# jimmyshe/liorf

Measured on AMD Instinct MI355X. Metric: LM iterations/sec (64-line scan vs 200k-pt map), higher is better.
Workload: dtype f32; 1 GPU; kitti64: 120000-pt scan vs 200000-pt local surf map, 30 LM iterations per scan (early exit off), one scan per GPU at a time, 8 distinct seeded scans in rotation, map replicated; n_q=120000, n_m=200000, distinct_scans=8, parallelism=scan-per-gpu x1

## Files before the change

include/liorf_s2m_debug.h:

```cpp
#ifndef LIORF_S2M_DEBUG_H
#define LIORF_S2M_DEBUG_H

#include "liorf_s2m.h"

#ifdef __cplusplus
extern "C" {
#endif

int  s2m_debug_device_trig(s2m_handle h, const float* x, size_t n, float* s, float* c, float* a);
int  s2m_debug_deferred(s2m_handle h, int slot);
int  s2m_time_iteration_kernel(s2m_handle h, const float pose[6], int reps, float* ms_per_launch);
int  s2m_time_iterations(s2m_handle h, const float pose[6], int reps, float* ms_per_iter, int cap);

int  s2m_time_loop_launches(s2m_handle h, const float pose[6], int reps, float* us_per_launch);

int  s2m_debug_time_steady(s2m_handle h, const float pose[6], int reps, int solve_prev, float* us_per_launch);

#define S2M_PROF_WORDS 32
int  s2m_debug_wave_profile(s2m_handle h, const float pose[6], int launches, uint64_t* out, size_t cap_waves);

int  s2m_debug_device_hypot(s2m_handle h, const float* x, const float* y, size_t n, float* r);

typedef struct s2m_debug_lm_close_out {
    float   AtA[36], AtB[6];
    int32_t n_sel_last;
    s2m_iter_trace trace;
    float   pose[6];
    float   pose_next[6];
    int32_t iters_run, converged, done, stalled, is_degenerate;
    int32_t n_rows_active;
    float   matP[36];
} s2m_debug_lm_close_out;
int  s2m_debug_lm_close(s2m_handle h, int form, int iter, const double* rows, int n_rows, const float pose0[6],
                        int degen_in, const float matP_in[36], s2m_debug_lm_close_out* out);
int  s2m_debug_lm_close_check_args(int form, int iter, int max_iter, const double* rows, int n_rows, const float pose0[6],
                                   const float matP_in[36], const s2m_debug_lm_close_out* out);

#define S2M_DEBUG_PREP_READ   (-1)
#define S2M_DEBUG_PREP_NEW    0
#define S2M_DEBUG_PREP_LEGACY 1
int  s2m_debug_scan_prep(s2m_handle h, int32_t chain, const float pose[6], int32_t* qperm, float* qxyz, int32_t* chunk_parts,
                         int32_t* chunk_factor, int32_t* wave_table, int32_t* n_waves);

#define S2M_ICP_RANGE 8
int  s2m_debug_icp_nearest(s2m_handle h, const void* src, size_t n_src, const void* tgt, size_t n_tgt, size_t stride_bytes, int32_t mode,
                           uint64_t* keys, int32_t* n_fallback);
int  s2m_debug_icp_time_nearest(s2m_handle h, const void* src, size_t n_src, const void* tgt, size_t n_tgt, size_t stride_bytes, int32_t mode,
                                int32_t reps, uint64_t* keys, int32_t* n_fallback, float* us_build, float* us_search);
int  s2m_debug_icp_align_device(s2m_handle h, const void* src, size_t n_src, const void* tgt, size_t n_tgt, size_t stride_bytes,
                                const s2m_icp_params* p , s2m_icp_result* out);
int  s2m_debug_icp_tuning(s2m_handle h, float cell_in_leaves, int32_t shell_cap, int32_t use_grid);

int  s2m_debug_pg_rebase(const double a_launch[12], const double a_now[12], double X[12]);

int  s2m_debug_pg_set_estimate(s2m_handle h, int32_t key, const double X[12]);
int  s2m_debug_pg_linearize(s2m_handle h, int32_t n_variables, int32_t n_extra, double* rc, double* Binv, double* Aof, double* Ji, double* Jj,
                            double* rx, double* ferr, double* fw, double* err, double* wmin);
#define S2M_DEBUG_PG_FWD 0
#define S2M_DEBUG_PG_BWD 1
#define S2M_DEBUG_PG_K   2
#define S2M_DEBUG_PG_KT  3
int  s2m_debug_pg_apply(s2m_handle h, int32_t op, int32_t cols, const double* in, double* out);
int  s2m_debug_pg_apply_check_args(int32_t n_variables, int32_t n_extra, int32_t op, int32_t cols, const double* in, const double* out);
typedef struct s2m_debug_pg_cg_out {
    double  rr, bb;
    int32_t iters, stop;
// ... 9 lines not shown
```

liorf_amd/csrc/s2m_abi_debug.hip:

```cpp
#include <hip/hip_runtime.h>

#include <cmath>
#include <cstring>
#include <algorithm>
#include <limits>
#include <vector>

#include "s2m_context.hpp"
#include "s2m_device.hpp"

using namespace s2m;
using namespace s2m::host;

namespace s2m {

__global__ __launch_bounds__(256) void k_debug_sincos(const float* __restrict__ x, int n, float* __restrict__ s, float* __restrict__ c,
                                                      float* __restrict__ a)
{
    const int i = blockIdx.x * blockDim.x + threadIdx.x;
    if (i < n) { s[i] = glibc_sincosf(x[i], 0); c[i] = glibc_sincosf(x[i], 1); if (a) a[i] = glibc_atanf(x[i]); }
}

__global__ __launch_bounds__(256) void k_debug_hypot(const float* __restrict__ x, const float* __restrict__ y, int n, float* __restrict__ r)
{
// ... 246 lines not shown
    }
    if ((!pose || chain == S2M_DEBUG_PREP_READ) && chunk_factor)
        S2M_HIP(h, hipMemcpyAsync(chunk_factor, h->reg.chunk_factor.p, sizeof(int32_t) * (size_t)n_chunks, hipMemcpyDeviceToHost, h->stream));
    if (qperm) S2M_HIP(h, hipMemcpyAsync(qperm, h->reg.qperm.p, sizeof(int32_t) * n, hipMemcpyDeviceToHost, h->stream));
    if (qxyz) {
        S2M_HIP(h, hipMemcpyAsync(qxyz, h->reg.qx.p, sizeof(float) * n, hipMemcpyDeviceToHost, h->stream));
        S2M_HIP(h, hipMemcpyAsync(qxyz + n, h->reg.qy.p, sizeof(float) * n, hipMemcpyDeviceToHost, h->stream));
        S2M_HIP(h, hipMemcpyAsync(qxyz + 2 * n, h->reg.qz.p, sizeof(float) * n, hipMemcpyDeviceToHost, h->stream));
    }
    if (chunk_parts) S2M_HIP(h, hipMemcpyAsync(chunk_parts, h->reg.chunk_parts.p, sizeof(int32_t) * (size_t)n_chunks, hipMemcpyDeviceToHost, h->stream));
    int32_t nw = 0;
    const bool have_table = !h->reg.table_stale;
    if (have_table) S2M_HIP(h, hipMemcpyAsync(&nw, h->reg.n_waves.p, sizeof(nw), hipMemcpyDeviceToHost, h->stream));
    S2M_HIP(h, hipStreamSynchronize(h->stream));
    if (nw < 0 || nw > h->hctx.table_cap) return fail(h, S2M_ERR_HIP, "wave count outside the table");
    if (wave_table && nw > 0) {
        S2M_HIP(h, hipMemcpyAsync(wave_table, h->reg.wave_table.p, sizeof(int2) * (size_t)nw, hipMemcpyDeviceToHost, h->stream));
        S2M_HIP(h, hipStreamSynchronize(h->stream));
    }
    if (n_waves) *n_waves = have_table ? nw : -1;
    return S2M_OK;
}

int s2m_debug_deferred(s2m_handle h, int slot)
{
    if (!h) return S2M_ERR_INVALID_ARG;
    if (slot >= 0) { if (slot >= (int)h->batch.kids.size()) return S2M_ERR_INVALID_ARG; h = h->batch.kids[(size_t)slot]; }
    return h->reg.h_state ? h->reg.h_state[1].deferred_total : 0;
}

static int time_iterations_impl(s2m_handle h, const float pose[6], int reps, float* ms_mean, float* ms_per_iter)
{
    if (!h || !pose || reps < 1) return S2M_ERR_INVALID_ARG;
    if (!h->reg.have_scan || h->reg.n_m == 0 || h->reg.n_q == 0) return fail(h, S2M_ERR_NO_SCAN, "needs a resident scan and map");
    S2M_HIP(h, hipSetDevice(h->device));
    int rc;
    if ((rc = upload_ctx(h))) return rc;
    const int nit = h->prm.max_iter;
    if (h->reg.iter_events.size() < (size_t)(2 * nit)) {
        const size_t old = h->reg.iter_events.size();
        h->reg.iter_events.resize(2 * nit);
        for (size_t k = old; k < h->reg.iter_events.size(); k++) S2M_HIP(h, hipEventCreate(&h->reg.iter_events[k]));
    }
    std::vector<double> per_iter((size_t)nit, 0.0);
    for (int rep = 0; rep < reps; rep++) {
        S2M_HIP(h, hipMemsetAsync(h->reg.cert.p, 0, sizeof(float4) * h->reg.n_q, h->stream));
// ... 88 lines not shown
```

liorf_amd/csrc/s2m_kernels.hpp:

```cpp
#pragma once
#include "s2m_device.hpp"

namespace s2m {

struct CtxHead { int32_t nblocks, n_q; const int2* wave_table; double* partials; const float *qx, *qy, *qz; float4 *cert, *plane_cache; };
struct StateHead { int32_t done, n_waves, isDegenerate, T_valid; float pose[6]; };
struct LmParams { int32_t min_corr, early_exit; double conv_deg, conv_cm; };
template <bool kPin = true>
__device__ __forceinline__ void load_heads(CtxP cp, gptr<DevState> st, int slot, CtxHead& c, StateHead& s, int& a0, int& a1)
{
    c.nblocks = cp->nblocks; c.n_q = cp->n_q; c.wave_table = cp->wave_table; c.partials = cp->partials;
    c.qx = cp->qx; c.qy = cp->qy; c.qz = cp->qz; c.cert = cp->cert; c.plane_cache = cp->plane_cache;
    s.done = st->done; s.n_waves = st->n_waves; s.isDegenerate = st->isDegenerate; s.T_valid = st->T_valid;
#pragma unroll
    for (int k = 0; k < 6; k++) s.pose[k] = st->pose2[slot][k];
    if (kPin)
    asm volatile("" : "+s"(c.nblocks), "+s"(c.n_q), "+s"(c.wave_table), "+s"(c.partials), "+s"(c.qx), "+s"(c.qy), "+s"(c.qz),
                      "+s"(c.cert), "+s"(c.plane_cache), "+s"(s.done), "+s"(s.n_waves), "+s"(s.isDegenerate), "+s"(s.T_valid),
                      "+s"(s.pose[0]), "+s"(s.pose[1]), "+s"(s.pose[2]), "+s"(s.pose[3]), "+s"(s.pose[4]), "+s"(s.pose[5]), "+s"(a0), "+s"(a1));
}
__device__ __forceinline__ LmParams lm_params(CtxP cp)
{
    LmParams p;
    p.min_corr = cp->min_corr; p.early_exit = cp->early_exit; p.conv_deg = cp->conv_deg; p.conv_cm = cp->conv_cm;
    return p;
}
__device__ __forceinline__ void swap_if(bool c, float& a, float& b)
{
    float t = a; a = c ? b : a; b = c ? t : b;
}
__device__ __forceinline__ void swap_if(bool c, int& a, int& b)
{
    int t = a; a = c ? b : a; b = c ? t : b;
}

__device__ __forceinline__ void chunk_table_body(const int32_t* __restrict__ parts, int n, int n_chunks, int capacity,
                                                 int2* __restrict__ table, int32_t* __restrict__ n_waves_out,
                                                 int32_t* __restrict__ factor, DevState* __restrict__ st)
{
    __shared__ int32_t wsum[16];
    __shared__ int32_t carry_s, tot_s[3], base_s, pol_s[9];
    const int lane = threadIdx.x & 63, wave = threadIdx.x >> 6;
    constexpr int kOnePerCu = 256 * (kBlock / 64);
    bool use_factor = factor != nullptr;
    if (use_factor) {
        int tb = 0, tf = 0;
        for (int c = threadIdx.x; c < n_chunks; c += 1024) { tb += min(8, parts[c]); tf += min(8, parts[c] * max(factor[c], 1)); }
#pragma unroll
        for (int off = 32; off > 0; off >>= 1) { tb += __shfl_xor(tb, off, 64); tf += __shfl_xor(tf, off, 64); }
        if (threadIdx.x == 0) { tot_s[0] = 0; base_s = 0; }
        __syncthreads();
        if (lane == 0) { atomicAdd(&base_s, tb); atomicAdd(&tot_s[0], tf); }
        __syncthreads();
        use_factor = !(base_s <= kOnePerCu && tot_s[0] > kOnePerCu);
        __syncthreads();
    }
    constexpr int kPolicies = 9;
    auto wish_under = [&](int c, int pol) {
        const int f = use_factor ? max(factor[c], 1) : 1;
        const bool heavy = f >= 8;
        const int fe = (pol == 0) ? f : ((pol == 1) ? (f >= 4 ? f : 1) : (heavy ? f : 1));
        const int w = min(8, parts[c] * fe);
        const int cap = (pol <= 2) ? 8 : ((pol <= 5) ? (heavy ? 8 : (32 >> pol)) : (256 >> pol));
        return min(w, cap);
    };
    int tp[kPolicies];
#pragma unroll
    for (int k = 0; k < kPolicies; k++) tp[k] = 0;
    for (int c = threadIdx.x; c < n_chunks; c += 1024) {
#pragma unroll
        for (int k = 0; k < kPolicies; k++) tp[k] += wish_under(c, k);
    }
#pragma unroll
    for (int k = 0; k < kPolicies; k++) {
#pragma unroll
        for (int off = 32; off > 0; off >>= 1) tp[k] += __shfl_xor(tp[k], off, 64);
    }
    if (threadIdx.x == 0) carry_s = 0;
    if (threadIdx.x < kPolicies) pol_s[threadIdx.x] = 0;
    __syncthreads();
    if (lane == 0) {
#pragma unroll
        for (int k = 0; k < kPolicies; k++) atomicAdd(&pol_s[k], tp[k]);
    }
    __syncthreads();
    const int cap_eff = capacity;
    int pol = kPolicies - 1;
#pragma unroll
    for (int k = kPolicies - 2; k >= 0; k--) if (pol_s[k] <= cap_eff) pol = k;
    auto wish = [&](int c) { return wish_under(c, pol); };
    constexpr int pcap = 8;
    for (int base = 0; base < n_chunks; base += 1024) {
        const int c = base + threadIdx.x;
        const int p = (c < n_chunks) ? min(wish(c), pcap) : 0;
        int incl = p;
#pragma unroll
        for (int off = 1; off < 64; off <<= 1) {
            const int o = __shfl_up(incl, off, 64);
            if (lane >= off) incl += o;
        }
        if (lane == 63) wsum[wave] = incl;
        __syncthreads();
        int woff = 0;
        for (int w = 0; w < wave; w++) woff += wsum[w];
        const int carry = carry_s;
        const int off0 = carry + woff + incl - p;
        if (c < n_chunks) {
            const int per = 64 / p;
            for (int j = 0; j < p; j++) {
                const int start = c * 64 + j * per;
                if (off0 + j < capacity) table[off0 + j] = make_int2(start, max(0, min(per, n - start)));
            }
        }
        __syncthreads();
        if (threadIdx.x == 1023) carry_s = carry + woff + incl;
        __syncthreads();
    }
    if (threadIdx.x == 0) {
        const int nw = min(carry_s, capacity);
        *n_waves_out = nw;
        if (st) st->n_waves = nw;
    }
    if (factor) for (int c = threadIdx.x; c < n_chunks; c += 1024) factor[c] = 0;
}

__global__ __launch_bounds__(1024) void k_chunk_table(const PrepTable tbl)
{
    const PrepSlot& ps = tbl.s[blockIdx.y];
    if (ps.n <= 0) return;
    chunk_table_body(ps.chunk_parts, ps.n, ps.n_chunks, ps.capacity, ps.wave_table, ps.n_waves, nullptr, nullptr);
    if (ps.stamps) {
        __syncthreads();
        if (threadIdx.x == 0) ps.stamps[1] = wall_clock64();
    }
}

__global__ __launch_bounds__(1024) void k_chunk_table_density(const SlotTable tbl)
{
    DevCtx* __restrict__ cp = const_cast<DevCtx*>(tbl.ctx[blockIdx.y]);
    DevState* __restrict__ st = tbl.st[blockIdx.y];
    if (!cp->density_pending) return;
    __syncthreads();
    if (threadIdx.x == 0) cp->density_pending = 0;
    chunk_table_body(cp->chunk_parts, cp->n_q, cp->n_chunks, cp->table_cap, cp->wave_table_rw, cp->n_waves_rw,
                     cp->chunk_factor, st);
}

__device__ __forceinline__ void plane_fit_5x3(float (&qr)[5][3], float (&x)[3])
{
    float hC[3], nU[3], nD[3];
    int perm[3] = { 0, 1, 2 };
#pragma unroll
    for (int k = 0; k < 3; k++) {
        float s = 0.0f;
#pragma unroll
        for (int i = 0; i < 5; i++) s += qr[i][k] * qr[i][k];
        nD[k] = sqrtf(s); nU[k] = nD[k];
    }
    float maxn = nU[0];
    if (nU[1] > maxn) maxn = nU[1];
    if (nU[2] > maxn) maxn = nU[2];
    const float th = maxn * FLT_EPSILON;
    const float threshold_helper = (th * th) / 5.0f;
    const float norm_downdate_threshold = sqrtf(FLT_EPSILON);
    int np = 3;

#pragma unroll
    for (int k = 0; k < 3; k++) {
// ... 406 lines not shown
    if (kFull && iter == 0) {
        __syncthreads();
        if (wave == 1 && lane == 0 && (int)sh.tot[27] >= lp.min_corr) {
            int degenerate = 0;
            if (!all_eigen_above(sh.AtA, cp->eig_thresh)) {
                for (int i = 0; i < 6; i++) for (int j = 0; j < 6; j++) sh.eA[i][j] = sh.AtA[i * 6 + j];
                eigen6_sym(sh.eA, sh.eV, sh.eW, sh.eR, sh.eC);
                for (int i = 0; i < 6; i++) for (int j = 0; j < 6; j++) sh.eV2[i][j] = sh.eV[i][j];
                for (int i = 5; i >= 0; i--) {
                    if (sh.eW[i] < cp->eig_thresh) { for (int j = 0; j < 6; j++) sh.eV2[i][j] = 0.0f; degenerate = 1; }
                    else break;
                }
                for (int i = 0; i < 6; i++) for (int j = 0; j < 6; j++) sh.eA[i][j] = sh.eV[i][j];
                inv6_lu(sh.eA, sh.eVi);
                for (int i = 0; i < 6; i++) for (int j = 0; j < 6; j++) {
                    double a = 0.0;
                    for (int k = 0; k < 6; k++) a += (double)sh.eVi[i][k] * (double)sh.eV2[k][j];
                    st->matP[i * 6 + j] = (float)a;
                }
            }
            st->isDegenerate = degenerate;
            __threadfence_block();
        }
        __syncthreads();
    }

    if (wave == 0) {
        if (n_sel < lp.min_corr) {
            if (t == 0) {
                if (writer) {
                    s2m_iter_trace tr;
                    tr.n_sel = n_sel; tr.stepped = 0; tr.deltaR = 0.0f; tr.deltaT = 0.0f;
#pragma unroll
                    for (int k = 0; k < 6; k++) { tr.pose[k] = pose0[k]; tr.delta[k] = 0.0f; st->pose[k] = pose0[k]; }
                    st->stalled = 1; st->done = 1;
                    st->iters_run = cp->max_iter;
                    store_trace(trace + iter, tr);
                }
#pragma unroll
                for (int k = 0; k < 6; k++) s_out[k] = pose0[k];
                s_out[6] = 1.0f;
            }
        } else {
            float colv[6], X[6];
#pragma unroll
            for (int i = 0; i < 6; i++) colv[i] = (lane < 6) ? sh.AtA[i * 6 + lane] : ((lane == 6) ? sh.AtB[i] : 0.0f);
            solve6_qr_lanes(lane, colv, X);
            if (stamps) stamps[2] = wall_clock64();
            if (t == 0) {
// ... 13 lines not shown
#pragma unroll
                for (int k = 0; k < 6; k++) { pose[k] += X[k]; s_out[k] = pose[k]; }
                const double r0 = (double)(X[0] * 57.29578f), r1 = (double)(X[1] * 57.29578f), r2 = (double)(X[2] * 57.29578f);
                const float deltaR = (float)sqrt(r0 * r0 + r1 * r1 + r2 * r2);
                const double t0 = (double)(X[3] * 100), t1 = (double)(X[4] * 100), t2 = (double)(X[5] * 100);
                const float deltaT = (float)sqrt(t0 * t0 + t1 * t1 + t2 * t2);
                const bool conv = ((double)deltaR < lp.conv_deg) && ((double)deltaT < lp.conv_cm);
                s_out[6] = (conv && lp.early_exit) ? 1.0f : 0.0f;
                if (writer) {
                    s2m_iter_trace tr;
                    tr.n_sel = n_sel; tr.stepped = 1; tr.deltaR = deltaR; tr.deltaT = deltaT;
#pragma unroll
                    for (int k = 0; k < 6; k++) { tr.delta[k] = X[k]; tr.pose[k] = pose[k]; }
#pragma unroll
                    for (int k = 0; k < 6; k++) { st->pose[k] = pose[k]; st->pose2[(iter + 1) & 1][k] = pose[k]; }
                    st->T_valid = 0;
                    store_trace(trace + iter, tr);
                    st->iters_run = iter + 1;
                    if (conv) st->converged = 1;
                    if (conv && lp.early_exit) st->done = 1;
                }
            }
        }
    }
    if (stamps) stamps[3] = wall_clock64();
    late();
    __syncthreads();
    if (stamps) stamps[4] = wall_clock64();
#pragma unroll
    for (int k = 0; k < 6; k++) pose_out[k] = s_out[k];
    return s_out[6] != 0.0f;
}

__global__ __launch_bounds__(256) void k_wave_density(const SlotTable tbl, int raw_limit)
{
    const CtxP cp = ctx_const(tbl.ctx[blockIdx.y]);
    const auto st = G((const DevState*)tbl.st[blockIdx.y]);
    const int lane = threadIdx.x & 63;
    const int wv = blockIdx.x * 4 + (threadIdx.x >> 6);
    if (!cp->density_pending || wv >= st->n_waves) return;
    const auto tb = G((const int2*)cp->wave_table);
    const int2 e = make_int2(tb[wv].x, tb[wv].y);
    const int i = e.x + lane;
    const bool valid = lane < e.y && i < cp->n_q;
    float sx = 0.0f, sy = 0.0f, sz = 0.0f;
    if (valid) {
// ... 215 lines not shown
```

liorf_amd/csrc/s2m_prep.hpp:

```cpp
#pragma once
#include "s2m_device.hpp"

namespace s2m {

__global__ __launch_bounds__(256) void k_bbox(const unsigned char* __restrict__ pts, size_t stride, int n, uint32_t* __restrict__ part)
{
    __shared__ float smn[4][3], smx[4][3];
    float mn[3] = { INFINITY, INFINITY, INFINITY }, mx[3] = { -INFINITY, -INFINITY, -INFINITY };
    for (int i = blockIdx.x * blockDim.x + threadIdx.x; i < n; i += gridDim.x * blockDim.x) {
        const float* p = reinterpret_cast<const float*>(pts + (size_t)i * stride);
#pragma unroll
        for (int d = 0; d < 3; d++) {
            float v = p[d];
            if (isfinite(v)) { mn[d] = fminf(mn[d], v); mx[d] = fmaxf(mx[d], v); }
        }
    }
#pragma unroll
    for (int d = 0; d < 3; d++) {
#pragma unroll
        for (int off = 32; off > 0; off >>= 1) {
            mn[d] = fminf(mn[d], __shfl_down(mn[d], off, 64));
            mx[d] = fmaxf(mx[d], __shfl_down(mx[d], off, 64));
        }
    }
// ... 108 lines not shown
    for (int k = t; k < kPolarCells; k += kPolarBlock) row[k] = hist[k];
}

__global__ __launch_bounds__(1024) void k_polar_prefix(const PrepTable tbl)
{
    const PrepSlot& ps = tbl.s[blockIdx.y];
    if (ps.n <= 0) return;
    int32_t* __restrict__ H = ps.block_hist; const int nb = ps.npb; int32_t* __restrict__ counts = ps.counts;
    __shared__ int32_t seg[16][64];
    const int lane = threadIdx.x & 63, s = threadIdx.x >> 6;
    const int col = blockIdx.x * 64 + lane;
    const int per = (nb + 15) / 16, b0 = min(s * per, nb), b1 = min(b0 + per, nb);
    int32_t sum = 0;
    for (int b = b0; b < b1; b++) sum += H[(size_t)b * kPolarCells + col];
    seg[s][lane] = sum;
    __syncthreads();
    int32_t run = 0, total = 0;
#pragma unroll
    for (int q = 0; q < 16; q++) { const int32_t v = seg[q][lane]; run += (q < s) ? v : 0; total += v; }
    if (s == 0) counts[col] = total;
    for (int b = b0; b < b1; b++) {
        const size_t at = (size_t)b * kPolarCells + col;
        const int32_t v = H[at];
        H[at] = run;
        run += v;
    }
}

__global__ __launch_bounds__(1024) void k_polar_scan(const PrepTable tbl)
{
    const PrepSlot& ps = tbl.s[blockIdx.y];
    if (ps.n <= 0) return;
    int32_t* __restrict__ counts = ps.counts; int32_t* __restrict__ start = ps.cell_start;
    __shared__ int32_t wsum[16];
    const int t = threadIdx.x, lane = t & 63, wave = t >> 6;
    int32_t v[16];
    int32_t sum = 0;
    int4* c4 = reinterpret_cast<int4*>(counts + t * 16);
#pragma unroll
    for (int k = 0; k < 4; k++) {
        const int4 q = c4[k];
        c4[k] = make_int4(0, 0, 0, 0);
        v[4 * k] = q.x; v[4 * k + 1] = q.y; v[4 * k + 2] = q.z; v[4 * k + 3] = q.w;
        sum += q.x + q.y + q.z + q.w;
    }
    int32_t incl = sum;
#pragma unroll
// ... 269 lines not shown
```

liorf_amd/s2m.py:

```python
from __future__ import annotations

import ctypes as C
import importlib.util
import os
import sys

import numpy as np

_HERE = os.path.dirname(os.path.abspath(__file__))
LIB_PATH = os.environ.get("S2M_LIB") or os.path.join(_HERE, "libliorf_s2m.so")

S2M_OK = 0
S2M_ERR_CAPACITY = -5
S2M_ERR_BUSY = -6
ERRORS = {-1: "S2M_ERR_INVALID_ARG", -2: "S2M_ERR_NO_DEVICE", -3: "S2M_ERR_HIP", -4: "S2M_ERR_NO_SCAN",
          -5: "S2M_ERR_CAPACITY", -6: "S2M_ERR_BUSY"}

ABI_SYMBOLS = [
    "s2m_version", "s2m_default_params", "s2m_create", "s2m_destroy", "s2m_last_error", "s2m_set_params", "s2m_get_params",
    "s2m_set_map", "s2m_set_map_device", "s2m_set_scan", "s2m_set_scan_device",
    "s2m_optimize", "s2m_optimize_resident", "s2m_optimize_launch", "s2m_optimize_collect",
    "s2m_optimize_batch", "s2m_batch_set_scan", "s2m_batch_set_scans", "s2m_slot_set_scan", "s2m_slot_optimize_launch", "s2m_slot_optimize_collect", "s2m_optimize_batch_launch", "s2m_optimize_batch_collect", "s2m_batch_get_trace",
    "s2m_get_trace", "s2m_surf_optimization", "s2m_normal_eq", "s2m_last_timing", "s2m_debug_deferred",
    "s2m_time_iteration_kernel", "s2m_time_iterations", "s2m_make_scancontext", "s2m_debug_wave_profile", "s2m_debug_time_steady", "s2m_time_loop_launches",
    "s2m_debug_scan_prep",
    "s2m_voxel_downsample", "s2m_voxel_downsample_device", "s2m_downsample_scan", "s2m_extract_cloud",
    "s2m_transform_cloud",
    "s2m_icp_default_params", "s2m_icp_align", "s2m_debug_device_trig", "s2m_debug_device_hypot",
    "s2m_debug_lm_close", "s2m_debug_lm_close_check_args",
    "s2m_sc_reset", "s2m_sc_size", "s2m_sc_add_scan", "s2m_sc_add_descriptor", "s2m_sc_detect_loop", "s2m_sc_distance",
    "s2m_sc_query_default_params", "s2m_sc_query_check_args", "s2m_sc_query_key", "s2m_sc_query_descriptor", "s2m_sc_query_scan", "s2m_sc_query_projected",
    "s2m_kf_default_params", "s2m_kf_reset", "s2m_kf_size", "s2m_kf_add", "s2m_kf_set_poses", "s2m_extract_surrounding",
    "s2m_loop_default_params", "s2m_loop_near_keyframes", "s2m_loop_align", "s2m_loop_closure_rs",
    "s2m_loop_align_launch", "s2m_loop_closure_rs_launch", "s2m_loop_poll", "s2m_loop_collect",
    "s2m_debug_icp_nearest", "s2m_debug_icp_time_nearest", "s2m_debug_icp_align_device", "s2m_debug_icp_tuning",
    "s2m_gmap_default_params", "s2m_global_map", "s2m_kf_map_cloud",
    "s2m_scan_layout_preset", "s2m_project_default_params", "s2m_imu_deskew_info", "s2m_project_check_args", "s2m_project_scan",
    "s2m_downsample_projected", "s2m_sc_add_projected",
    "s2m_odom_deskew_info", "s2m_project_check_args_motion", "s2m_project_scan_motion", "s2m_guess_state_init", "s2m_update_initial_guess",
    "s2m_pg_default_params", "s2m_pg_check_args", "s2m_pg_reset", "s2m_pg_size", "s2m_pg_add_prior", "s2m_pg_add_between", "s2m_pg_add_gps",
    "s2m_pg_set_initial", "s2m_pg_add_odometry", "s2m_pg_optimize", "s2m_pg_get_poses", "s2m_pg_marginal", "s2m_pg_apply_to_store",
    "s2m_pg_marginals_check_args", "s2m_pg_marginals", "s2m_pg_joint_marginal",
    "s2m_pg_optimize_launch", "s2m_pg_optimize_poll", "s2m_pg_optimize_collect", "s2m_debug_pg_rebase",
    "s2m_debug_pg_set_estimate", "s2m_debug_pg_linearize", "s2m_debug_pg_apply", "s2m_debug_pg_apply_check_args", "s2m_debug_pg_cg",
    "s2m_debug_pg_retract",
]
S2M_RING_U8, S2M_RING_U16, S2M_RING_I32 = 0, 1, 2
S2M_TIME_F32, S2M_TIME_U32_NS, S2M_TIME_U32, S2M_TIME_F64_REL = 0, 1, 2, 3
# ... 195 lines not shown
    L.s2m_optimize_launch.argtypes = [vp, fp]
    L.s2m_optimize_collect.argtypes = [vp, fp, C.POINTER(ImuInit), C.POINTER(Result)]
    L.s2m_get_trace.argtypes = [vp, C.POINTER(IterTrace), C.c_int]
    L.s2m_optimize_batch.argtypes = [vp, C.c_int, C.POINTER(vp), C.POINTER(C.c_size_t), C.c_size_t, fp, C.POINTER(ImuInit), C.POINTER(Result)]
    L.s2m_batch_set_scan.argtypes = [vp, C.c_int, vp, C.c_size_t, C.c_size_t, C.c_int]
    L.s2m_slot_set_scan.argtypes = [vp, C.c_int, vp, C.c_size_t, C.c_size_t, C.c_int]
    L.s2m_slot_optimize_launch.argtypes = [vp, C.c_int, fp]
    L.s2m_slot_optimize_collect.argtypes = [vp, C.c_int, fp, C.POINTER(ImuInit), C.POINTER(Result)]
    L.s2m_batch_set_scans.argtypes = [vp, C.c_int, C.POINTER(C.c_void_p), C.POINTER(C.c_size_t), C.c_size_t, C.c_int]
    L.s2m_optimize_batch_launch.argtypes = [vp, C.c_int, fp]
    L.s2m_optimize_batch_collect.argtypes = [vp, C.c_int, fp, C.POINTER(ImuInit), C.POINTER(Result)]
    L.s2m_batch_get_trace.argtypes = [vp, C.c_int, C.POINTER(IterTrace), C.c_int]
    L.s2m_surf_optimization.argtypes = [vp, fp, C.POINTER(C.c_int32), fp, C.POINTER(C.c_uint8), fp]
    L.s2m_normal_eq.argtypes = [vp, fp, fp, fp, C.POINTER(C.c_int32)]
    L.s2m_last_timing.argtypes = [vp, fp, fp, fp]
    L.s2m_debug_deferred.argtypes = [vp, C.c_int]
    L.s2m_time_iteration_kernel.argtypes = [vp, fp, C.c_int, fp]
    L.s2m_time_iterations.argtypes = [vp, fp, C.c_int, fp, C.c_int]
    L.s2m_debug_wave_profile.argtypes = [vp, fp, C.c_int, C.POINTER(C.c_uint64), C.c_size_t]
    L.s2m_debug_time_steady.argtypes = [vp, fp, C.c_int, C.c_int, fp]
    L.s2m_time_loop_launches.argtypes = [vp, fp, C.c_int, fp]
    L.s2m_debug_scan_prep.argtypes = [vp, C.c_int32, fp, C.POINTER(C.c_int32), fp, C.POINTER(C.c_int32), C.POINTER(C.c_int32),
                                      C.POINTER(C.c_int32), C.POINTER(C.c_int32)]
    L.s2m_make_scancontext.argtypes = [vp, vp, C.c_size_t, C.c_size_t, C.POINTER(C.c_double), C.POINTER(C.c_double)]
    szp = C.POINTER(C.c_size_t)
    for n in ("s2m_voxel_downsample", "s2m_voxel_downsample_device"):
        getattr(L, n).argtypes = [vp, vp, C.c_size_t, C.c_size_t, C.c_float, vp, C.c_size_t, C.c_size_t, szp]
    L.s2m_downsample_scan.argtypes = [vp, vp, C.c_size_t, C.c_size_t, C.c_int, C.c_float, vp, C.c_size_t, C.c_size_t, szp]
    L.s2m_extract_cloud.argtypes = [vp, C.c_int, C.POINTER(vp), szp, C.c_size_t, C.c_int, fp, C.c_float,
                                    vp, C.c_size_t, C.c_size_t, szp]
    L.s2m_transform_cloud.argtypes = [vp, vp, C.c_size_t, C.c_size_t, fp, vp, C.c_size_t]
    dp, i32p = C.POINTER(C.c_double), C.POINTER(C.c_int32)
    L.s2m_debug_device_trig.argtypes = [vp, fp, C.c_size_t, fp, fp, fp]
    L.s2m_debug_device_hypot.argtypes = [vp, fp, fp, C.c_size_t, fp]
    L.s2m_debug_lm_close.argtypes = [vp, C.c_int, C.c_int, dp, C.c_int, fp, C.c_int, fp, C.POINTER(LmCloseOut)]
    L.s2m_debug_lm_close_check_args.argtypes = [C.c_int, C.c_int, C.c_int, dp, C.c_int, fp, fp, C.POINTER(LmCloseOut)]
    L.s2m_icp_default_params.argtypes = [C.POINTER(IcpParams)]
    L.s2m_icp_align.argtypes = [vp, vp, C.c_size_t, vp, C.c_size_t, C.c_size_t, C.POINTER(IcpParams), C.POINTER(IcpResult)]
    L.s2m_sc_reset.argtypes = [vp]
    L.s2m_sc_size.argtypes = [vp]
    L.s2m_sc_add_scan.argtypes = [vp, vp, C.c_size_t, C.c_size_t]
    L.s2m_sc_add_descriptor.argtypes = [vp, dp]
    L.s2m_sc_detect_loop.argtypes = [vp, i32p, fp, C.POINTER(ScMatch)]
    L.s2m_sc_distance.argtypes = [vp, C.c_int32, i32p, C.c_int32, dp, i32p]
    qp, hp = C.POINTER(ScQueryParams), C.POINTER(ScHit)
    L.s2m_sc_query_default_params.argtypes = [qp]
# ... 418 lines not shown
        p = np.ascontiguousarray(pose0, np.float32).reshape(6)
        m = np.ascontiguousarray(matP_in, np.float32).reshape(36)
        out = LmCloseOut()
        self._check(self.lib.s2m_debug_lm_close(self.h, form, it, r.ctypes.data_as(C.POINTER(C.c_double)), r.shape[0], _fp(p),
                                                int(degen_in), _fp(m), C.byref(out)), "s2m_debug_lm_close")
        return out

    def scanPrep(self, chain: int = 0, pose=None) -> dict:
        n = self.laserCloudSurfLastDSNum
        nc = (n + 63) // 64
        i32 = C.POINTER(C.c_int32)
        qperm = np.zeros(n, np.int32)
        qxyz = np.zeros((3, n), np.float32)
        parts, factor = np.zeros(nc, np.int32), np.zeros(nc, np.int32)
        table = np.zeros((nc * 12 + 64, 2), np.int32)
        nw = C.c_int32(0)
        p = None if pose is None else np.ascontiguousarray(pose, np.float32)
        self._check(self.lib.s2m_debug_scan_prep(self.h, int(chain), None if p is None else _fp(p), qperm.ctypes.data_as(i32), _fp(qxyz),
                                                 parts.ctypes.data_as(i32), factor.ctypes.data_as(i32), table.ctypes.data_as(i32),
                                                 C.byref(nw)), "s2m_debug_scan_prep")
        return dict(qperm=qperm, qxyz=qxyz, chunk_parts=parts, chunk_factor=factor, wave_table=table[:max(nw.value, 0)].copy(),
                    n_waves=nw.value)

    def timing(self):
        a, b, c = C.c_float(0), C.c_float(0), C.c_float(0)
        self.lib.s2m_last_timing(self.h, C.byref(a), C.byref(b), C.byref(c))
        return dict(optimize_ms=a.value, set_map_ms=b.value, set_scan_ms=c.value)

    def time_iteration_kernel(self, pose, reps: int = 200) -> float:
        p = np.ascontiguousarray(pose, np.float32)
        ms = C.c_float(0)
        self._check(self.lib.s2m_time_iteration_kernel(self.h, _fp(p), reps, C.byref(ms)), "s2m_time_iteration_kernel")
        return ms.value

    def time_iterations(self, pose, reps: int = 10) -> np.ndarray:
        p = np.ascontiguousarray(pose, np.float32)
        out = np.zeros(64, np.float32)
        self._check(self.lib.s2m_time_iterations(self.h, _fp(p), reps, _fp(out), 64), "s2m_time_iterations")
        return out[:self.params.max_iter]

    def time_loop_launches(self, pose, reps: int = 10) -> float:
        p = np.ascontiguousarray(pose, np.float32)
        us = C.c_float(0)
        self._check(self.lib.s2m_time_loop_launches(self.h, _fp(p), reps, C.byref(us)), "s2m_time_loop_launches")
        return us.value

# ... 655 lines not shown
```

Before: 56380 LM iterations/s.

## Rewrite chunk wave-table builder as register-blocked single-pass scan with DPP reductions

The chunk-to-wave table kernel is restructured so each thread owns a contiguous run of chunks held in registers. All policy sums are computed in one pass, reduced across waves with DPP row scans, and the table is written without the per-1024 carry loop and its repeated block barriers. The density variant loads context fields into scalars up front and clears the pending flag inside the body. The LM close path for the full variant gets a separate branch that solves on wave 0 and applies the pose update from thread 0, only syncing on the first iteration. It also tweaks a polar histogram prefix write and adds a debug entry point for testing the table builder, at the cost of more complex code and possible ordering risks around the skipped barrier.

```diff
diff --git a/include/liorf_s2m_debug.h b/include/liorf_s2m_debug.h
--- a/include/liorf_s2m_debug.h
+++ b/include/liorf_s2m_debug.h
@@ -42,6 +42,11 @@
 int  s2m_debug_scan_prep(s2m_handle h, int32_t chain, const float pose[6], int32_t* qperm, float* qxyz, int32_t* chunk_parts,
                          int32_t* chunk_factor, int32_t* wave_table, int32_t* n_waves);
 
+int  s2m_debug_chunk_table(s2m_handle h, const int32_t* parts, const int32_t* factor, int32_t n_chunks, int32_t n, int32_t capacity,
+                           int32_t pending, int32_t* table, int32_t* n_waves, int32_t* state_n_waves, int32_t* factor_out,
+                           int32_t* pending_out);
+int  s2m_debug_chunk_table_check_args(const int32_t* parts, int32_t n_chunks, int32_t n, int32_t capacity, const int32_t* table);
+
 #define S2M_ICP_RANGE 8
 int  s2m_debug_icp_nearest(s2m_handle h, const void* src, size_t n_src, const void* tgt, size_t n_tgt, size_t stride_bytes, int32_t mode,
                            uint64_t* keys, int32_t* n_fallback);
diff --git a/liorf_amd/csrc/s2m_abi_debug.hip b/liorf_amd/csrc/s2m_abi_debug.hip
--- a/liorf_amd/csrc/s2m_abi_debug.hip
+++ b/liorf_amd/csrc/s2m_abi_debug.hip
@@ -292,6 +292,76 @@
     return S2M_OK;
 }
 
+int s2m_debug_chunk_table_check_args(const int32_t* parts, int32_t n_chunks, int32_t n, int32_t capacity, const int32_t* table)
+{
+    if (!parts || !table || n < 1 || n_chunks != (n + 63) / 64 || capacity < 1 || capacity > (1 << 24)) return S2M_ERR_INVALID_ARG;
+    for (int32_t c = 0; c < n_chunks; c++) if (parts[c] < 1 || parts[c] > 8) return S2M_ERR_INVALID_ARG;
+    return S2M_OK;
+}
+
+int s2m_debug_chunk_table(s2m_handle h, const int32_t* parts, const int32_t* factor, int32_t n_chunks, int32_t n, int32_t capacity,
+                          int32_t pending, int32_t* table, int32_t* n_waves, int32_t* state_n_waves, int32_t* factor_out,
+                          int32_t* pending_out)
+{
+    if (!h) return S2M_ERR_INVALID_ARG;
+    if (s2m_debug_chunk_table_check_args(parts, n_chunks, n, capacity, table))
+        return fail(h, S2M_ERR_INVALID_ARG, "null parts / table, n < 1, n_chunks other than n / 64 rounded up, capacity outside 1 .. 2^24, or a part outside 1 .. 8");
+    if (factor) for (int32_t c = 0; c < n_chunks; c++)
+        if (factor[c] < 0 || factor[c] > 8) return fail(h, S2M_ERR_INVALID_ARG, "a density wish outside 0 .. 8");
+    S2M_HIP(h, hipSetDevice(h->device));
+    const size_t nc = (size_t)n_chunks, sz_parts = sizeof(int32_t) * nc, sz_table = sizeof(int2) * (size_t)capacity;
+    void* dev[6] = { nullptr, nullptr, nullptr, nullptr, nullptr, nullptr };
+    const size_t sizes[6] = { sz_parts, sz_parts, sz_table, sizeof(int32_t), sizeof(DevCtx), sizeof(DevState) };
+    auto release = [&]() { for (void* p : dev) if (p) (void)hipFree(p); };
+    for (int k = 0; k < 6; k++)
+        if (hipMalloc(&dev[k], sizes[k]) != hipSuccess) { release(); return fail(h, S2M_ERR_HIP, "hipMalloc (s2m_debug_chunk_table)"); }
+    int32_t *d_parts = (int32_t*)dev[0], *d_factor = (int32_t*)dev[1], *d_nw = (int32_t*)dev[3];
+    int2* d_table = (int2*)dev[2];
+    DevCtx* d_ctx = (DevCtx*)dev[4];
+    DevState* d_st = (DevState*)dev[5];
+    DevCtx c;
+    memset(&c, 0, sizeof(c));
+    c.n_q = n; c.n_chunks = n_chunks; c.table_cap = capacity; c.density_pending = pending;
+    c.chunk_parts = d_parts; c.chunk_factor = d_factor; c.wave_table_rw = d_table; c.n_waves_rw = d_nw;
+    c.wave_table = d_table; c.n_waves = d_nw; c.state = d_st;
+    hipError_t e = hipMemcpyAsync(d_parts, parts, sz_parts, hipMemcpyHostToDevice, h->stream);
+    if (e == hipSuccess) e = factor ? hipMemcpyAsync(d_factor, factor, sz_parts, hipMemcpyHostToDevice, h->stream) : hipMemsetAsync(d_factor, 0, sz_parts, h->stream);
+    if (e == hipSuccess) e = hipMemsetAsync(d_table, 0xff, sz_table, h->stream);
+    if (e == hipSuccess) e = hipMemsetAsync(d_nw, 0xff, sizeof(int32_t), h->stream);
+    if (e == hipSuccess) e = hipMemsetAsync(d_st, 0xff, sizeof(DevState), h->stream);
+    if (e == hipSuccess) e = hipMemcpyAsync(d_ctx, &c, sizeof(c), hipMemcpyHostToDevice, h->stream);
+    if (e == hipSuccess) e = hipStreamSynchronize(h->stream);
+    if (e == hipSuccess) {
+        if (factor) {
+            LoopShape sh;
+            memset(&sh.tbl, 0, sizeof(sh.tbl));
+            sh.tbl.ctx[0] = d_ctx; sh.tbl.st[0] = d_st;
+            sh.nslots = 1; sh.table_cap = capacity;
+            launch_density_table(h, sh);
+        } else {
+            PrepTable t;
+            memset(&t, 0, sizeof(t));
+            t.s[0].n = n; t.s[0].n_chunks = n_chunks; t.s[0].capacity = capacity;
+            t.s[0].chunk_parts = d_parts; t.s[0].wave_table = d_table; t.s[0].n_waves = d_nw;
+            launch_chunk_table(h->stream, t, 1);
+        }
+        e = hipGetLastError();
+    }
+    int32_t st_nw = -1;
+    DevCtx back;
+    if (e == hipSuccess) e = hipMemcpyAsync(table, d_table, sz_table, hipMemcpyDeviceToHost, h->stream);
+    if (e == hipSuccess && n_waves) e = hipMemcpyAsync(n_waves, d_nw, sizeof(int32_t), hipMemcpyDeviceToHost, h->stream);
+    if (e == hipSuccess) e = hipMemcpyAsync(&st_nw, &d_st->n_waves, sizeof(int32_t), hipMemcpyDeviceToHost, h->stream);
+    if (e == hipSuccess && factor_out) e = hipMemcpyAsync(factor_out, d_factor, sz_parts, hipMemcpyDeviceToHost, h->stream);
+    if (e == hipSuccess) e = hipMemcpyAsync(&back, d_ctx, sizeof(back), hipMemcpyDeviceToHost, h->stream);
+    if (e == hipSuccess) e = hipStreamSynchronize(h->stream);
+    release();
+    if (e != hipSuccess) return fail(h, S2M_ERR_HIP, "s2m_debug_chunk_table", e);
+    if (state_n_waves) *state_n_waves = st_nw;
+    if (pending_out) *pending_out = back.density_pending;
+    return S2M_OK;
+}
+
 int s2m_debug_deferred(s2m_handle h, int slot)
 {
     if (!h) return S2M_ERR_INVALID_ARG;
diff --git a/liorf_amd/csrc/s2m_kernels.hpp b/liorf_amd/csrc/s2m_kernels.hpp
--- a/liorf_amd/csrc/s2m_kernels.hpp
+++ b/liorf_amd/csrc/s2m_kernels.hpp
@@ -34,101 +34,141 @@
     int t = a; a = c ? b : a; b = c ? t : b;
 }
 
-__device__ __forceinline__ void chunk_table_body(const int32_t* __restrict__ parts, int n, int n_chunks, int capacity,
-                                                 int2* __restrict__ table, int32_t* __restrict__ n_waves_out,
-                                                 int32_t* __restrict__ factor, DevState* __restrict__ st)
-{
-    __shared__ int32_t wsum[16];
-    __shared__ int32_t carry_s, tot_s[3], base_s, pol_s[9];
-    const int lane = threadIdx.x & 63, wave = threadIdx.x >> 6;
+constexpr int kTableRegs = 8;
+constexpr int kTableSums = 13;
+constexpr int kTablePolicies = 9;
+constexpr int kTableRow = 17;
+typedef int v2i __attribute__((ext_vector_type(2)));
+__device__ __forceinline__ int table_wish(int p, int f, int pol)
+{
+    const bool heavy = f >= 8;
+    const int fe = (pol == 0) ? f : ((pol == 1) ? (f >= 4 ? f : 1) : (heavy ? f : 1));
+    const int w = min(8, p * fe);
+    const int cap = (pol <= 2) ? 8 : ((pol <= 5) ? (heavy ? 8 : (32 >> pol)) : (256 >> pol));
+    return min(w, cap);
+}
+__device__ __forceinline__ constexpr int table_plain_sum(int pol) { return pol <= 2 ? 0 : 1 + (pol - 3) % 3; }
+__device__ __forceinline__ int row_incl_scan_i32(int v)
+{
+    v += dpp_i32<0x111, 0xf>(0, v); v += dpp_i32<0x112, 0xf>(0, v);
+    v += dpp_i32<0x114, 0xf>(0, v); v += dpp_i32<0x118, 0xf>(0, v);
+    return v;
+}
+template <int NT, bool kRegs>
+__device__ __forceinline__ void chunk_table_impl(gptr<const int32_t> parts, int n, int n_chunks, int capacity,
+                                                 gptr<int2> table, gptr<int32_t> n_waves_out, gptr<int32_t> factor,
+                                                 gptr<DevState> st, gptr<int32_t> flag, bool go, int32_t (*wsum)[kTableRow])
+{
+    constexpr int NW = NT / 64;
+    static_assert(NT % 64 == 0 && NW <= 16, "the wave sums are scanned across the 16 lanes of one DPP row");
+    const int t = threadIdx.x, lane = t & 63, wave = __builtin_amdgcn_readfirstlane(t >> 6);
     constexpr int kOnePerCu = 256 * (kBlock / 64);
-    bool use_factor = factor != nullptr;
-    if (use_factor) {
-        int tb = 0, tf = 0;
-        for (int c = threadIdx.x; c < n_chunks; c += 1024) { tb += min(8, parts[c]); tf += min(8, parts[c] * max(factor[c], 1)); }
-#pragma unroll
-        for (int off = 32; off > 0; off >>= 1) { tb += __shfl_xor(tb, off, 64); tf += __shfl_xor(tf, off, 64); }
-        if (threadIdx.x == 0) { tot_s[0] = 0; base_s = 0; }
-        __syncthreads();
-        if (lane == 0) { atomicAdd(&base_s, tb); atomicAdd(&tot_s[0], tf); }
-        __syncthreads();
-        use_factor = !(base_s <= kOnePerCu && tot_s[0] > kOnePerCu);
-        __syncthreads();
-    }
-    constexpr int kPolicies = 9;
-    auto wish_under = [&](int c, int pol) {
-        const int f = use_factor ? max(factor[c], 1) : 1;
-        const bool heavy = f >= 8;
-        const int fe = (pol == 0) ? f : ((pol == 1) ? (f >= 4 ? f : 1) : (heavy ? f : 1));
-        const int w = min(8, parts[c] * fe);
-        const int cap = (pol <= 2) ? 8 : ((pol <= 5) ? (heavy ? 8 : (32 >> pol)) : (256 >> pol));
-        return min(w, cap);
+    const bool has_f = factor != nullptr;
+    const int k = (n_chunks + NT - 1) / NT;
+    const int c0 = t * k;
+    const int kk = kRegs ? kTableRegs : k;
+    int pr[kTableRegs], fr[kTableRegs];
+    if (kRegs) {
+#pragma unroll
+        for (int i = 0; i < kTableRegs; i++) {
+            const int c = c0 + i;
+            const bool own = i < k && c < n_chunks;
+            pr[i] = own ? parts[c] : 0;
+            fr[i] = (own && has_f) ? factor[c] : 0;
+        }
+#pragma unroll
+        for (int i = 0; i < kTableRegs; i++) asm volatile("" : "+v"(pr[i]), "+v"(fr[i]));
+    }
+    if (!go) return;
+    auto part_of = [&](int i) { const int c = c0 + i; return kRegs ? pr[i] : ((i < k && c < n_chunks) ? parts[c] : 0); };
+    auto fact_of = [&](int i) { const int c = c0 + i; return kRegs ? fr[i] : ((i < k && c < n_chunks && has_f) ? factor[c] : 0); };
+    auto for_own = [&](auto&& fn) __attribute__((always_inline)) {
+        constexpr int U = kRegs ? kTableRegs : 1;
+        for (int i0 = 0; i0 < kk; i0 += U) {
+#pragma unroll
+            for (int u = 0; u < U; u++) if (i0 + u < k) fn(i0 + u);
+        }
     };
-    int tp[kPolicies];
-#pragma unroll
-    for (int k = 0; k < kPolicies; k++) tp[k] = 0;
-    for (int c = threadIdx.x; c < n_chunks; c += 1024) {
-#pragma unroll
-        for (int k = 0; k < kPolicies; k++) tp[k] += wish_under(c, k);
-    }
-#pragma unroll
-    for (int k = 0; k < kPolicies; k++) {
-#pragma unroll
-        for (int off = 32; off > 0; off >>= 1) tp[k] += __shfl_xor(tp[k], off, 64);
-    }
-    if (threadIdx.x == 0) carry_s = 0;
-    if (threadIdx.x < kPolicies) pol_s[threadIdx.x] = 0;
+    int sm[kTableSums];
+#pragma unroll
+    for (int j = 0; j < kTableSums; j++) sm[j] = 0;
+    for_own([&](int i) {
+        const int p = part_of(i), f = max(fact_of(i), 1);
+        sm[0] += table_wish(p, 1, 0); sm[1] += table_wish(p, 1, 3); sm[2] += table_wish(p, 1, 4); sm[3] += table_wish(p, 1, 5);
+        if (has_f) {
+#pragma unroll
+            for (int q = 0; q < kTablePolicies; q++) sm[4 + q] += table_wish(p, f, q);
+        }
+    });
+#pragma unroll
+    for (int j = 0; j < kTableSums; j++) {
+        if (j < 4 || has_f) {
+            const int tot = __builtin_amdgcn_readlane(wave_incl_scan_i32(sm[j]), 63);
+            if (lane == 0) wsum[wave][j] = tot;
+        }
+    }
     __syncthreads();
-    if (lane == 0) {
-#pragma unroll
-        for (int k = 0; k < kPolicies; k++) atomicAdd(&pol_s[k], tp[k]);
-    }
-    __syncthreads();
-    const int cap_eff = capacity;
-    int pol = kPolicies - 1;
-#pragma unroll
-    for (int k = kPolicies - 2; k >= 0; k--) if (pol_s[k] <= cap_eff) pol = k;
-    auto wish = [&](int c) { return wish_under(c, pol); };
+    if (flag && t == 0) *flag = 0;
+    int ws[kTableSums], tot[kTableSums];
+#pragma unroll
+    for (int j = 0; j < kTableSums; j++) {
+        ws[j] = 0; tot[j] = 0;
+        if (j < 4 || has_f) {
+            ws[j] = row_incl_scan_i32(lane < NW ? wsum[lane][j] : 0);
+            tot[j] = __builtin_amdgcn_readlane(ws[j], NW - 1);
+        }
+    }
+    const bool use_factor = has_f && !(tot[0] <= kOnePerCu && tot[4] > kOnePerCu);
+    int pol = kTablePolicies - 1;
+#pragma unroll
+    for (int q = kTablePolicies - 2; q >= 0; q--) if ((use_factor ? tot[4 + q] : tot[table_plain_sum(q)]) <= capacity) pol = q;
+    const int sel = use_factor ? 4 + pol : table_plain_sum(pol);
+    int wsel = ws[0];
+#pragma unroll
+    for (int j = 1; j < kTableSums; j++) wsel = (sel == j) ? ws[j] : wsel;
+    const int total = __builtin_amdgcn_readlane(wsel, NW - 1);
+    const int woff = wave > 0 ? __builtin_amdgcn_readlane(wsel, wave - 1) : 0;
     constexpr int pcap = 8;
-    for (int base = 0; base < n_chunks; base += 1024) {
-        const int c = base + threadIdx.x;
-        const int p = (c < n_chunks) ? min(wish(c), pcap) : 0;
-        int incl = p;
-#pragma unroll
-        for (int off = 1; off < 64; off <<= 1) {
-            const int o = __shfl_up(incl, off, 64);
-            if (lane >= off) incl += o;
-        }
-        if (lane == 63) wsum[wave] = incl;
-        __syncthreads();
-        int woff = 0;
-        for (int w = 0; w < wave; w++) woff += wsum[w];
-        const int carry = carry_s;
-        const int off0 = carry + woff + incl - p;
-        if (c < n_chunks) {
-            const int per = 64 / p;
+    int own = 0;
+    for_own([&](int i) { own += min(table_wish(part_of(i), use_factor ? max(fact_of(i), 1) : 1, pol), pcap); });
+    int off0 = woff + wave_incl_scan_i32(own) - own;
+    const auto table2 = (gptr<v2i>)table;
+    for_own([&](int i) {
+        const int c = c0 + i;
+        const int p = min(table_wish(part_of(i), use_factor ? max(fact_of(i), 1) : 1, pol), pcap);
+        if (p > 0) {
+            const int per = (int)((0x08090A0C10152040ull >> ((p - 1) * 8)) & 0xffu);
             for (int j = 0; j < p; j++) {
                 const int start = c * 64 + j * per;
-                if (off0 + j < capacity) table[off0 + j] = make_int2(start, max(0, min(per, n - start)));
-            }
-        }
-        __syncthreads();
-        if (threadIdx.x == 1023) carry_s = carry + woff + incl;
-        __syncthreads();
-    }
-    if (threadIdx.x == 0) {
-        const int nw = min(carry_s, capacity);
+                if (off0 + j < capacity) table2[off0 + j] = v2i{ start, max(0, min(per, n - start)) };
+            }
+        }
+        off0 += p;
+    });
+    if (t == 0) {
+        const int nw = min(total, capacity);
         *n_waves_out = nw;
         if (st) st->n_waves = nw;
     }
-    if (factor) for (int c = threadIdx.x; c < n_chunks; c += 1024) factor[c] = 0;
+    if (has_f) {
+        for_own([&](int i) { const int c = c0 + i; if (i < k && c < n_chunks) factor[c] = 0; });
+    }
+}
+template <int NT>
+__device__ __forceinline__ void chunk_table_body(gptr<const int32_t> parts, int n, int n_chunks, int capacity,
+                                                 gptr<int2> table, gptr<int32_t> n_waves_out, gptr<int32_t> factor,
+                                                 gptr<DevState> st, gptr<int32_t> flag = nullptr, bool go = true)
+{
+    __shared__ int32_t wsum[NT / 64][kTableRow];
+    if (n_chunks <= NT * kTableRegs) chunk_table_impl<NT, true>(parts, n, n_chunks, capacity, table, n_waves_out, factor, st, flag, go, wsum);
+    else                             chunk_table_impl<NT, false>(parts, n, n_chunks, capacity, table, n_waves_out, factor, st, flag, go, wsum);
 }
 
 __global__ __launch_bounds__(1024) void k_chunk_table(const PrepTable tbl)
 {
     const PrepSlot& ps = tbl.s[blockIdx.y];
     if (ps.n <= 0) return;
-    chunk_table_body(ps.chunk_parts, ps.n, ps.n_chunks, ps.capacity, ps.wave_table, ps.n_waves, nullptr, nullptr);
+    chunk_table_body<1024>(G((const int32_t*)ps.chunk_parts), ps.n, ps.n_chunks, ps.capacity, G(ps.wave_table), G(ps.n_waves), nullptr, nullptr);
     if (ps.stamps) {
         __syncthreads();
         if (threadIdx.x == 0) ps.stamps[1] = wall_clock64();
@@ -137,13 +177,14 @@
 
 __global__ __launch_bounds__(1024) void k_chunk_table_density(const SlotTable tbl)
 {
-    DevCtx* __restrict__ cp = const_cast<DevCtx*>(tbl.ctx[blockIdx.y]);
-    DevState* __restrict__ st = tbl.st[blockIdx.y];
-    if (!cp->density_pending) return;
-    __syncthreads();
-    if (threadIdx.x == 0) cp->density_pending = 0;
-    chunk_table_body(cp->chunk_parts, cp->n_q, cp->n_chunks, cp->table_cap, cp->wave_table_rw, cp->n_waves_rw,
-                     cp->chunk_factor, st);
+    const CtxP cp = ctx_const(tbl.ctx[blockIdx.y]);
+    const auto st = G(tbl.st[blockIdx.y]);
+    int pending = cp->density_pending, n = cp->n_q, n_chunks = cp->n_chunks, cap = cp->table_cap;
+    const int32_t* parts = cp->chunk_parts; int32_t* factor = cp->chunk_factor;
+    int2* table = cp->wave_table_rw; int32_t* n_waves = cp->n_waves_rw;
+    asm volatile("" : "+s"(pending), "+s"(n), "+s"(n_chunks), "+s"(cap), "+s"(parts), "+s"(factor), "+s"(table), "+s"(n_waves));
+    chunk_table_body<1024>(G(parts), n, n_chunks, cap, G(table), G(n_waves), G(factor), st,
+                           G(&const_cast<DevCtx*>(tbl.ctx[blockIdx.y])->density_pending), pending != 0);
 }
 
 __device__ __forceinline__ void plane_fit_5x3(float (&qr)[5][3], float (&x)[3])
@@ -596,9 +637,9 @@
             st->isDegenerate = degenerate;
             __threadfence_block();
         }
-        __syncthreads();
-    }
-
+    }
+
+    if constexpr (!kFull) {
     if (wave == 0) {
         if (n_sel < lp.min_corr) {
             if (t == 0) {
@@ -658,6 +699,75 @@
                 }
             }
         }
+    }
+    } else {
+        auto update = [&](float (&X)[6]) __attribute__((always_inline)) {
+            float pose[6];
+#pragma unroll
+            for (int k = 0; k < 6; k++) pose[k] = pose0[k];
+            if ((iter == 0) ? (st->isDegenerate != 0) : (degen0 != 0)) {
+                float X2[6];
+#pragma unroll
+                for (int k = 0; k < 6; k++) X2[k] = X[k];
+                for (int i = 0; i < 6; i++) {
+                    double a = 0.0;
+                    for (int k = 0; k < 6; k++) a += (double)st->matP[i * 6 + k] * (double)X2[k];
+                    X[i] = (float)a;
+                }
+            }
+#pragma unroll
+            for (int k = 0; k < 6; k++) { pose[k] += X[k]; s_out[k] = pose[k]; }
+            const double r0 = (double)(X[0] * 57.29578f), r1 = (double)(X[1] * 57.29578f), r2 = (double)(X[2] * 57.29578f);
+            const float deltaR = (float)sqrt(r0 * r0 + r1 * r1 + r2 * r2);
+            const double t0 = (double)(X[3] * 100), t1 = (double)(X[4] * 100), t2 = (double)(X[5] * 100);
+            const float deltaT = (float)sqrt(t0 * t0 + t1 * t1 + t2 * t2);
+            const bool conv = ((double)deltaR < lp.conv_deg) && ((double)deltaT < lp.conv_cm);
+            s_out[6] = (conv && lp.early_exit) ? 1.0f : 0.0f;
+            if (writer) {
+                s2m_iter_trace tr;
+                tr.n_sel = n_sel; tr.stepped = 1; tr.deltaR = deltaR; tr.deltaT = deltaT;
+#pragma unroll
+                for (int k = 0; k < 6; k++) { tr.delta[k] = X[k]; tr.pose[k] = pose[k]; }
+#pragma unroll
+                for (int k = 0; k < 6; k++) { st->pose[k] = pose[k]; st->pose2[(iter + 1) & 1][k] = pose[k]; }
+                st->T_valid = 0;
+                store_trace(trace + iter, tr);
+                st->iters_run = iter + 1;
+                if (conv) st->converged = 1;
+                if (conv && lp.early_exit) st->done = 1;
+            }
+        };
+        float Xf[6];
+        bool solved = false;
+        if (wave == 0) {
+            if (n_sel < lp.min_corr) {
+                if (t == 0) {
+                    if (writer) {
+                        s2m_iter_trace tr;
+                        tr.n_sel = n_sel; tr.stepped = 0; tr.deltaR = 0.0f; tr.deltaT = 0.0f;
+#pragma unroll
+                        for (int k = 0; k < 6; k++) { tr.pose[k] = pose0[k]; tr.delta[k] = 0.0f; st->pose[k] = pose0[k]; }
+                        st->stalled = 1; st->done = 1;
+                        st->iters_run = cp->max_iter;
+                        store_trace(trace + iter, tr);
+                    }
+#pragma unroll
+                    for (int k = 0; k < 6; k++) s_out[k] = pose0[k];
+                    s_out[6] = 1.0f;
+                }
+            } else {
+                float colv[6], X[6];
+#pragma unroll
+                for (int i = 0; i < 6; i++) colv[i] = (lane < 6) ? sh.AtA[i * 6 + lane] : ((lane == 6) ? sh.AtB[i] : 0.0f);
+                solve6_qr_lanes(lane, colv, X);
+                if (stamps) stamps[2] = wall_clock64();
+                solved = true;
+#pragma unroll
+                for (int k = 0; k < 6; k++) Xf[k] = X[k];
+            }
+        }
+        if (iter == 0) __syncthreads();
+        if (solved && t == 0) update(Xf);
     }
     if (stamps) stamps[3] = wall_clock64();
     late();
diff --git a/liorf_amd/csrc/s2m_prep.hpp b/liorf_amd/csrc/s2m_prep.hpp
--- a/liorf_amd/csrc/s2m_prep.hpp
+++ b/liorf_amd/csrc/s2m_prep.hpp
@@ -154,7 +154,7 @@
     for (int b = b0; b < b1; b++) {
         const size_t at = (size_t)b * kPolarCells + col;
         const int32_t v = H[at];
-        H[at] = run;
+        if (v > 0) H[at] = run;
         run += v;
     }
 }
diff --git a/liorf_amd/s2m.py b/liorf_amd/s2m.py
--- a/liorf_amd/s2m.py
+++ b/liorf_amd/s2m.py
@@ -23,7 +23,7 @@
     "s2m_optimize_batch", "s2m_batch_set_scan", "s2m_batch_set_scans", "s2m_slot_set_scan", "s2m_slot_optimize_launch", "s2m_slot_optimize_collect", "s2m_optimize_batch_launch", "s2m_optimize_batch_collect", "s2m_batch_get_trace",
     "s2m_get_trace", "s2m_surf_optimization", "s2m_normal_eq", "s2m_last_timing", "s2m_debug_deferred",
     "s2m_time_iteration_kernel", "s2m_time_iterations", "s2m_make_scancontext", "s2m_debug_wave_profile", "s2m_debug_time_steady", "s2m_time_loop_launches",
-    "s2m_debug_scan_prep",
+    "s2m_debug_scan_prep", "s2m_debug_chunk_table", "s2m_debug_chunk_table_check_args",
     "s2m_voxel_downsample", "s2m_voxel_downsample_device", "s2m_downsample_scan", "s2m_extract_cloud",
     "s2m_transform_cloud",
     "s2m_icp_default_params", "s2m_icp_align", "s2m_debug_device_trig", "s2m_debug_device_hypot",
@@ -265,6 +265,8 @@
     L.s2m_time_loop_launches.argtypes = [vp, fp, C.c_int, fp]
     L.s2m_debug_scan_prep.argtypes = [vp, C.c_int32, fp, C.POINTER(C.c_int32), fp, C.POINTER(C.c_int32), C.POINTER(C.c_int32),
                                       C.POINTER(C.c_int32), C.POINTER(C.c_int32)]
+    L.s2m_debug_chunk_table.argtypes = [vp, C.POINTER(C.c_int32), C.POINTER(C.c_int32), C.c_int32, C.c_int32, C.c_int32, C.c_int32] + [C.POINTER(C.c_int32)] * 5
+    L.s2m_debug_chunk_table_check_args.argtypes = [C.POINTER(C.c_int32), C.c_int32, C.c_int32, C.c_int32, C.POINTER(C.c_int32)]
     L.s2m_make_scancontext.argtypes = [vp, vp, C.c_size_t, C.c_size_t, C.POINTER(C.c_double), C.POINTER(C.c_double)]
     szp = C.POINTER(C.c_size_t)
     for n in ("s2m_voxel_downsample", "s2m_voxel_downsample_device"):
@@ -729,6 +731,20 @@
         return dict(qperm=qperm, qxyz=qxyz, chunk_parts=parts, chunk_factor=factor, wave_table=table[:max(nw.value, 0)].copy(),
                     n_waves=nw.value)
 
+    def chunkTable(self, parts, factor, n: int, capacity: int, pending: int = 1) -> dict:
+        i32 = C.POINTER(C.c_int32)
+        pa = np.ascontiguousarray(parts, np.int32)
+        fa = None if factor is None else np.ascontiguousarray(factor, np.int32)
+        assert fa is None or fa.shape == pa.shape
+        table = np.zeros((max(int(capacity), 0), 2), np.int32)
+        fout = np.zeros(pa.shape[0], np.int32)
+        nw, snw, pend = C.c_int32(0), C.c_int32(0), C.c_int32(0)
+        self._check(self.lib.s2m_debug_chunk_table(self.h, pa.ctypes.data_as(i32), None if fa is None else fa.ctypes.data_as(i32),
+                                                   pa.shape[0], int(n), int(capacity), int(pending), table.ctypes.data_as(i32),
+                                                   C.byref(nw), C.byref(snw), fout.ctypes.data_as(i32), C.byref(pend)),
+                    "s2m_debug_chunk_table")
+        return dict(table=table, n_waves=nw.value, state_n_waves=snw.value, factor=fout, pending=pend.value)
+
     def timing(self):
         a, b, c = C.c_float(0), C.c_float(0), C.c_float(0)
         self.lib.s2m_last_timing(self.h, C.byref(a), C.byref(b), C.byref(c))
```

Measured after the change: 57060 LM iterations/s, median of 5. 1.01x the previous value.
